# facebookresearch/NasRec

Hardware: AMD Instinct MI355X
Metric: supernet samples/sec at batch 256 (Criteo-shape), 1/2/4/8 MI355X (higher is better)
Workload: dtype f32

## Files before the change

nasrec_amd/csrc/gemm_kslice.hip:

```cpp
#include <cstdlib>
#include <cstring>
#include "gemm_tile.h"

#define KS_TM 32
#define KS_TN 32
#define KS_DC 128
#define KS_NB 4
#define KS_CH ((KS_TM + KS_TN) * KS_DC)
#define KS_SEGS 4
#ifdef KS_STAMPS
#define KS_STAMP(i) \
  if (tid == 0 && d.workspace) d.workspace[blockIdx.x * 64 + (i)] = __builtin_bit_cast(float, (unsigned)__builtin_readcyclecounter())
#define KS_LOOP_STAMP_A const unsigned ks_ta = (unsigned)__builtin_readcyclecounter()
#define KS_LOOP_STAMP_B ks_wait += (unsigned)__builtin_readcyclecounter() - ks_ta
#else
#define KS_STAMP(i)
#define KS_LOOP_STAMP_A
#define KS_LOOP_STAMP_B
#endif

__device__ __forceinline__ __amdgpu_buffer_rsrc_t ks_rsrc(const float* p, long floats) {
  return __builtin_amdgcn_make_buffer_rsrc(const_cast<float*>(p), 0, (int)(floats <= 0 ? 0 : (floats > 0x1fffffffL ? 0x7fffffffL : 4 * floats)), 0x00020000);
}

__global__ __launch_bounds__(1024) void gemm_kslice_kernel(const nasrec_gemm_desc_t d, int tiles_m_, int tiles_n_) {
  extern __shared__ __attribute__((aligned(16))) float ks_lds[];
  const int tid = threadIdx.x, lane = tid & 63;
  KS_STAMP(0);
  warm_kernarg<1024>();
  const int wave = __builtin_amdgcn_readfirstlane(tid >> 6);
#ifndef KS_FEED_FIRST
#define KS_FEED_FIRST 1
#endif
  const int rw = KS_FEED_FIRST ? (wave ^ 8) : wave;
  const int tile = rw & 3;
  const int tm = tile >> 1, tn = tile & 1;
  const int fr = lane & 15, fg = lane >> 4;
  typedef int i32x2 __attribute__((ext_vector_type(2)));
  typedef int i32x4 __attribute__((ext_vector_type(4)));
  i32x4 ab[KS_SEGS], mnkl[KS_SEGS];
  i32x2 ll[KS_SEGS], tiles;
  int nseg;
  {
    const unsigned long long ka = (unsigned long long)__builtin_amdgcn_kernarg_segment_ptr();
    constexpr int S0 = offsetof(nasrec_gemm_desc_t, seg), SS = sizeof(nasrec_gemm_seg_t), OM = offsetof(nasrec_gemm_seg_t, M),
                  OL = offsetof(nasrec_gemm_seg_t, ldb);
    static_assert(KS_SEGS == 4 && offsetof(nasrec_gemm_seg_t, B) == 8 && offsetof(nasrec_gemm_seg_t, lda) == OM + 12 &&
                      offsetof(nasrec_gemm_seg_t, ldc) == OL + 4 && sizeof(nasrec_gemm_desc_t) % 8 == 0,
                  "descriptor layout the scalar loads below assume");
    asm volatile(
        "s_load_dword %12, %14, %c15\n"
        "s_load_dwordx2 %13, %14, %c16\n"
        "s_load_dwordx4 %0, %14, %c17\n"
        "s_load_dwordx4 %1, %14, %c18\n"
        "s_load_dwordx4 %2, %14, %c19\n"
        "s_load_dwordx4 %3, %14, %c20\n"
        "s_load_dwordx4 %4, %14, %c21\n"
        "s_load_dwordx4 %5, %14, %c22\n"
        "s_load_dwordx4 %6, %14, %c23\n"
        "s_load_dwordx4 %7, %14, %c24\n"
        "s_load_dwordx2 %8, %14, %c25\n"
        "s_load_dwordx2 %9, %14, %c26\n"
        "s_load_dwordx2 %10, %14, %c27\n"
        "s_load_dwordx2 %11, %14, %c28\n"
        "s_waitcnt lgkmcnt(0)"
        : "=&s"(ab[0]), "=&s"(ab[1]), "=&s"(ab[2]), "=&s"(ab[3]), "=&s"(mnkl[0]), "=&s"(mnkl[1]), "=&s"(mnkl[2]), "=&s"(mnkl[3]),
          "=&s"(ll[0]), "=&s"(ll[1]), "=&s"(ll[2]), "=&s"(ll[3]), "=&s"(nseg), "=&s"(tiles)
        : "s"(ka), "n"(offsetof(nasrec_gemm_desc_t, nseg)), "n"(sizeof(nasrec_gemm_desc_t)), "n"(S0), "n"(S0 + SS), "n"(S0 + 2 * SS),
          "n"(S0 + 3 * SS), "n"(S0 + OM), "n"(S0 + SS + OM), "n"(S0 + 2 * SS + OM), "n"(S0 + 3 * SS + OM), "n"(S0 + OL),
          "n"(S0 + SS + OL), "n"(S0 + 2 * SS + OL), "n"(S0 + 3 * SS + OL)
        : "memory");
  }
  const float* sA[KS_SEGS];
  const float* sB[KS_SEGS];
  int sK[KS_SEGS], sLa[KS_SEGS], sLb[KS_SEGS], sN[KS_SEGS];
#pragma unroll
  for (int q = 0; q < KS_SEGS; ++q) {
    sA[q] = reinterpret_cast<const float*>(((unsigned long long)(unsigned)ab[q][1] << 32) | (unsigned)ab[q][0]);
    sB[q] = reinterpret_cast<const float*>(((unsigned long long)(unsigned)ab[q][3] << 32) | (unsigned)ab[q][2]);
    sK[q] = mnkl[q][2];
    sLa[q] = mnkl[q][3];
    sLb[q] = ll[q][0];
  }
  const nasrec_gemm_seg_t& s0 = d.seg[0];
  const int M = mnkl[0][0], N = mnkl[0][1];
  const int tiles_m = tiles[0], tiles_n = tiles[1];
  const int nwg = tiles_m * tiles_n, lin0 = blockIdx.x;
  const int q8 = nwg >> 3, r8 = nwg & 7, xcd = lin0 & 7;
  const int lin = (xcd < r8 ? xcd * (q8 + 1) : r8 * (q8 + 1) + (xcd - r8) * q8) + (lin0 >> 3);
  const int PM = tiles_m < 4 ? tiles_m : 4;
  const int panel = lin / (PM * tiles_n), within = lin - panel * PM * tiles_n;
  const int ph = min(PM, tiles_m - panel * PM);
  const int bx = within / ph, by = panel * PM + (within - bx * ph);
  const int m0 = by * KS_TM, n0 = bx * KS_TN;

  int nchunks = 0, ntiny = 0, sT[KS_SEGS];
#pragma unroll
  for (int q = 0; q < KS_SEGS; ++q) {
    const bool live = (q < nseg) & (sA[q] != nullptr) & (sK[q] > 0);
    sK[q] = live ? sK[q] : 0;
    const bool tiny = (sK[q] > 0) & (sK[q] <= 16) & (ntiny < 2);
    sT[q] = tiny ? sK[q] : 0;
    sK[q] = tiny ? 0 : sK[q];
    ntiny += tiny ? 1 : 0;
    sN[q] = (sK[q] + KS_DC - 1) / KS_DC;
    nchunks += sN[q];
  }
  const bool feeder = rw >= 8;
  float* red = ks_lds;
  if (feeder) {
    const int f = rw - 8;
    const bool isB = f >= 4;
    const int pslot = lane & 31;
    int grow[4], gkg[4], growld[4];
#pragma unroll
    for (int i = 0; i < 4; ++i) {
      const int row = 2 * (4 * f + i) + (lane >> 5);
      gkg[i] = pslot ^ (row & 15);
      grow[i] = isB ? min(n0 + row - 32, N - 1) : min(m0 + row, M - 1);
    }
    auto next_live = [&](int seg) {
      int r = KS_SEGS;
#pragma unroll
      for (int q = KS_SEGS - 1; q >= 0; --q) r = (q > seg && sK[q] > 0) ? q : r;
      return r;
    };
    const float* iP;
    int iseg = next_live(-1), iK, ild, ik0 = 0, ibuf = 0;
    __amdgpu_buffer_rsrc_t irs;
    auto issue_segment = [&]() {
      iP = nullptr, iK = 0, ild = 0;
#pragma unroll
      for (int q = 0; q < KS_SEGS; ++q) {
        const bool here = iseg == q;
        iP = here ? (isB ? sB[q] : sA[q]) : iP;
        iK = here ? sK[q] : iK;
        ild = here ? (isB ? sLb[q] : sLa[q]) : ild;
      }
      irs = ks_rsrc(iP, iK > 0 ? (long)((isB ? N : M) - 1) * ild + iK : 0);
#pragma unroll
      for (int i = 0; i < 4; ++i) growld[i] = grow[i] * ild;
    };
    issue_segment();
    auto issue = [&]() {
#pragma unroll
      for (int i = 0; i < 4; ++i) {
        const int k = ik0 + 4 * gkg[i];
        const int vo = k < iK ? 4 * (growld[i] + k) : 0x7ffffff0;
        float* dst = ks_lds + ibuf * KS_CH + (4 * f + i) * 256;
        __builtin_amdgcn_raw_ptr_buffer_load_lds(irs, (__attribute__((address_space(3))) void*)dst, 16, vo, 0, 0, 0);
      }
      ibuf = ibuf + 1 == KS_NB ? 0 : ibuf + 1;
      ik0 += KS_DC;
      if (ik0 >= iK && iseg < KS_SEGS) {
        iseg = next_live(iseg);
        ik0 = 0;
        issue_segment();
      }
    };
#pragma unroll
    for (int c = 0; c < KS_NB - 1; ++c) issue();
#ifdef KS_STAMPS
    unsigned fw_data = 0, fw_bar = 0, fw_issue = 0;
#endif
    for (int c = 0; c < nchunks; ++c) {
#ifdef KS_STAMPS
      const unsigned ta = (unsigned)__builtin_readcyclecounter();
#endif
      asm volatile("s_waitcnt vmcnt(8)" ::: "memory");
#ifdef KS_STAMPS
      const unsigned tb = (unsigned)__builtin_readcyclecounter();
#endif
      __builtin_amdgcn_s_barrier();
#ifdef KS_STAMPS
      const unsigned tc = (unsigned)__builtin_readcyclecounter();
#endif
      issue();
#ifdef KS_STAMPS
      const unsigned td = (unsigned)__builtin_readcyclecounter();
      fw_data += tb - ta, fw_bar += tc - tb, fw_issue += td - tc;
#endif
    }
#ifdef KS_STAMPS
    if (lane == 0 && d.workspace) {
      d.workspace[blockIdx.x * 64 + 16 + wave * 3 + 0] = __builtin_bit_cast(float, fw_data);
      d.workspace[blockIdx.x * 64 + 16 + wave * 3 + 1] = __builtin_bit_cast(float, fw_bar);
      d.workspace[blockIdx.x * 64 + 16 + wave * 3 + 2] = __builtin_bit_cast(float, fw_issue);
    }
#endif
    KS_STAMP(4);
    asm volatile("s_waitcnt vmcnt(0)" ::: "memory");
    __builtin_amdgcn_s_barrier();
  } else {
    const int half = rw >> 2;
#ifdef KS_STAMPS
    unsigned ks_wait = 0;
    const unsigned ks_t0 = (unsigned)__builtin_readcyclecounter();
#endif
    f32x4 acc0 = {0.f, 0.f, 0.f, 0.f}, acc1 = {0.f, 0.f, 0.f, 0.f};
    f32x4 fa[2][4], fb[2][4];
    int flim[2];
    int ck = 0, cbuf = 0;
    int cseg = 0, cK = 0;
    auto seg_k = [&](int seg) {
      int K = 0;
#pragma unroll
      for (int q = 0; q < KS_SEGS; ++q) K = seg == q ? sK[q] : K;
      return K;
    };
    while (cseg < KS_SEGS && seg_k(cseg) == 0) ++cseg;
    cK = seg_k(cseg);
    f32x4 ta = {0.f, 0.f, 0.f, 0.f}, tb = {0.f, 0.f, 0.f, 0.f};
    int tK = 0;
    {
      const float *tA = nullptr, *tB = nullptr;
      int tla = 0, tlb = 0, seen = 0;
#pragma unroll
      for (int q = 0; q < KS_SEGS; ++q) {
        const bool tiny = sT[q] > 0;
        const bool mine = tiny & (seen == half);
        tA = mine ? sA[q] : tA;
        tB = mine ? sB[q] : tB;
        tla = mine ? sLa[q] : tla;
        tlb = mine ? sLb[q] : tlb;
        tK = mine ? sT[q] : tK;
        seen += tiny ? 1 : 0;
      }
      if (tK > 0) {
        const __amdgpu_buffer_rsrc_t ra = ks_rsrc(tA, (long)(M - 1) * tla + tK), rb = ks_rsrc(tB, (long)(N - 1) * tlb + tK);
        const int ia = min(m0 + tm * 16 + fr, M - 1), ib = min(n0 + tn * 16 + fr, N - 1);
        ta = __builtin_bit_cast(f32x4, __builtin_amdgcn_raw_buffer_load_b128(ra, 4 * (ia * tla + 4 * fg), 0, 0));
        tb = __builtin_bit_cast(f32x4, __builtin_amdgcn_raw_buffer_load_b128(rb, 4 * (ib * tlb + 4 * fg), 0, 0));
      }
    }
    auto readfrag = [&](int set) {
      const float* buf = ks_lds + cbuf * KS_CH;
      flim[set] = cK - ck;
#pragma unroll
      for (int kb = 0; kb < 4; ++kb) {
        const int g = 16 * half + 4 * kb + fg;
        fa[set][kb] = *reinterpret_cast<const f32x4*>(buf + (tm * 16 + fr) * KS_DC + 4 * (g ^ fr));
        fb[set][kb] = *reinterpret_cast<const f32x4*>(buf + (32 + tn * 16 + fr) * KS_DC + 4 * (g ^ fr));
      }
      cbuf = cbuf + 1 == KS_NB ? 0 : cbuf + 1;
      ck += KS_DC;
      if (ck >= cK) {
        do {
          ++cseg;
        } while (cseg < KS_SEGS && seg_k(cseg) == 0);
        ck = 0;
        cK = seg_k(cseg);
      }
    };
    auto multiply = [&](int set) {
      const int lim = flim[set];
      if (lim < KS_DC) {
#pragma unroll
        for (int kb = 0; kb < 4; ++kb)
#pragma unroll
          for (int e = 0; e < 4; ++e) {
            const bool in = 4 * (16 * half + 4 * kb + fg) + e < lim;
            fa[set][kb][e] = in ? fa[set][kb][e] : 0.f;
            fb[set][kb][e] = in ? fb[set][kb][e] : 0.f;
          }
      }
#pragma unroll
      for (int kb = 0; kb < 4; kb += 2)
#pragma unroll
        for (int j = 0; j < 4; ++j) {
          acc0 = __builtin_amdgcn_mfma_f32_16x16x4f32(fa[set][kb][j], fb[set][kb][j], acc0, 0, 0, 0);
          acc1 = __builtin_amdgcn_mfma_f32_16x16x4f32(fa[set][kb + 1][j], fb[set][kb + 1][j], acc1, 0, 0, 0);
        }
    };
    for (int t = 0; t < nchunks + 1; t += 2) {
#pragma unroll
      for (int h = 0; h < 2; ++h) {
        const int c = t + h;
        if (c < nchunks) {
          asm volatile("s_waitcnt lgkmcnt(0)" ::: "memory");
          KS_LOOP_STAMP_A;
          __builtin_amdgcn_s_barrier();
          KS_LOOP_STAMP_B;
          readfrag(h);
        }
        if (c >= 1 && c <= nchunks) multiply(h ^ 1);
      }
    }
    KS_STAMP(4);
    asm volatile("s_waitcnt lgkmcnt(0)" ::: "memory");
    __builtin_amdgcn_s_barrier();
    if (tK > 0) {
#pragma unroll
      for (int e = 0; e < 4; ++e) {
        const bool in = 4 * fg + e < tK;
        ta[e] = in ? ta[e] : 0.f;
        tb[e] = in ? tb[e] : 0.f;
      }
#pragma unroll
      for (int j = 0; j < 4; ++j) acc0 = __builtin_amdgcn_mfma_f32_16x16x4f32(ta[j], tb[j], acc0, 0, 0, 0);
    }
    const f32x4 acc = acc0 + acc1;
#ifdef KS_STAMPS
    if (lane == 0 && d.workspace) {
      d.workspace[blockIdx.x * 64 + 16 + wave * 3 + 1] = __builtin_bit_cast(float, ks_wait);
      d.workspace[blockIdx.x * 64 + 16 + wave * 3 + 2] = __builtin_bit_cast(float, (unsigned)__builtin_readcyclecounter() - ks_t0);
    }
#endif
    *reinterpret_cast<f32x4*>(&red[((half * 4 + tile) * 64 + lane) * 4]) = acc;
  }
  __syncthreads();
  KS_STAMP(5);
  {
    const int e = wave;
    const int etile = e >> 2, r = e & 3;
    const float v = red[((0 * 4 + etile) * 64 + lane) * 4 + r] + red[((1 * 4 + etile) * 64 + lane) * 4 + r];
    const int i = m0 + (etile >> 1) * 16 + 4 * fg + r, j = n0 + (etile & 1) * 16 + fr;
    if (i < M && j < N) epilogue_store<NASREC_CM_PLAIN>(d, s0, i, j, v);
  }
  KS_STAMP(6);
}

bool gemm_kslice_eligible(const nasrec_gemm_desc_t* d) {
  if (d->amode != NASREC_AM_KC || d->bmode != NASREC_AM_KC || d->cmode != NASREC_CM_PLAIN || d->zmode || d->splitk > 1) return false;
  if (d->nseg > KS_SEGS) return false;
  const nasrec_gemm_seg_t& s0 = d->seg[0];
  long K = 0;
  for (int q = 0; q < d->nseg; ++q) {
    const nasrec_gemm_seg_t& s = d->seg[q];
    if (s.Aaux || s.Baux || s.ones_col || (s.Mvalid > 0 && s.Mvalid < s0.M)) return false;
    if (s.A && s.K > 0) {
      K += s.K;
      if ((long)s0.M * s.lda >= (1L << 29) || (long)s0.N * s.ldb >= (1L << 29)) return false;
    }
  }
  const long tiles = (long)((s0.M + KS_TM - 1) / KS_TM) * ((s0.N + KS_TN - 1) / KS_TN);
  return s0.M <= 512 && tiles >= 128 && tiles <= 512 && K >= 512;
}

int launch_gemm_kslice(hipStream_t st, const nasrec_gemm_desc_t* d) {
  const nasrec_gemm_seg_t& s0 = d->seg[0];
  const int tiles_m = (s0.M + KS_TM - 1) / KS_TM, tiles_n = (s0.N + KS_TN - 1) / KS_TN;
  static unsigned long long attr_devices = 0;
  const size_t lds = sizeof(float) * KS_NB * KS_CH;
  if (nasrec_lds_attr_needed(attr_devices))
    (void)hipFuncSetAttribute(reinterpret_cast<const void*>(&gemm_kslice_kernel), hipFuncAttributeMaxDynamicSharedMemorySize, (int)lds);
  hipLaunchKernelGGL(gemm_kslice_kernel, dim3((unsigned)(tiles_m * tiles_n)), dim3(1024), lds, st, *d, tiles_m, tiles_n);
  return nasrec_check_launch("gemm_kslice");
}
```

Baseline: 1.160 million.

## Reshape k-slice GEMM tile to 16x48 with one feeder SIMD and four-way K split

Changes the workgroup tile from 32x32 to 16x48 and remaps the 16 waves by SIMD: the waves on SIMD 0 feed A/B chunks into LDS with eight loads each, and each of the other three SIMDs owns one 16x16 output tile whose K range is split four ways across its waves. The final reduction sums four partials per output tile, and the rasterization panel height grows to 8. The aim is to spread MFMA work evenly across SIMDs and shrink the load each feeder wave carries. In exchange each workgroup loads more B per output element, there are fewer MFMAs per wave per chunk, and the deeper vmcnt wait changes how loads overlap. Eligibility still counts 32x32 tiles even though the launch grid now uses 16x48 tiles.

```diff
diff --git a/nasrec_amd/csrc/gemm_kslice.hip b/nasrec_amd/csrc/gemm_kslice.hip
--- a/nasrec_amd/csrc/gemm_kslice.hip
+++ b/nasrec_amd/csrc/gemm_kslice.hip
@@ -2,8 +2,11 @@
 #include <cstring>
 #include "gemm_tile.h"
 
-#define KS_TM 32
-#define KS_TN 32
+#define KS_TM 16
+#define KS_TN 48
+#define KS_NT (KS_TN / 16)
+#define KS_PPF 8
+#define KS_PANEL 8
 #define KS_DC 128
 #define KS_NB 4
 #define KS_CH ((KS_TM + KS_TN) * KS_DC)
@@ -29,12 +32,11 @@
   KS_STAMP(0);
   warm_kernarg<1024>();
   const int wave = __builtin_amdgcn_readfirstlane(tid >> 6);
-#ifndef KS_FEED_FIRST
-#define KS_FEED_FIRST 1
-#endif
-  const int rw = KS_FEED_FIRST ? (wave ^ 8) : wave;
-  const int tile = rw & 3;
-  const int tm = tile >> 1, tn = tile & 1;
+#ifndef KS_SIMD_MAP
+#define KS_SIMD_MAP 0
+#endif
+  const int simd = KS_SIMD_MAP ? (wave >> 2) : (wave & 3), slot = KS_SIMD_MAP ? (wave & 3) : (wave >> 2);
+  const int tile = simd - 1;
   const int fr = lane & 15, fg = lane >> 4;
   typedef int i32x2 __attribute__((ext_vector_type(2)));
   typedef int i32x4 __attribute__((ext_vector_type(4)));
@@ -88,7 +90,7 @@
   const int nwg = tiles_m * tiles_n, lin0 = blockIdx.x;
   const int q8 = nwg >> 3, r8 = nwg & 7, xcd = lin0 & 7;
   const int lin = (xcd < r8 ? xcd * (q8 + 1) : r8 * (q8 + 1) + (xcd - r8) * q8) + (lin0 >> 3);
-  const int PM = tiles_m < 4 ? tiles_m : 4;
+  const int PM = tiles_m < KS_PANEL ? tiles_m : KS_PANEL;
   const int panel = lin / (PM * tiles_n), within = lin - panel * PM * tiles_n;
   const int ph = min(PM, tiles_m - panel * PM);
   const int bx = within / ph, by = panel * PM + (within - bx * ph);
@@ -106,18 +108,18 @@
     sN[q] = (sK[q] + KS_DC - 1) / KS_DC;
     nchunks += sN[q];
   }
-  const bool feeder = rw >= 8;
+  const bool feeder = simd == 0;
   float* red = ks_lds;
   if (feeder) {
-    const int f = rw - 8;
-    const bool isB = f >= 4;
+    const int f = slot;
+    const bool isB = f >= 1;
     const int pslot = lane & 31;
-    int grow[4], gkg[4], growld[4];
-#pragma unroll
-    for (int i = 0; i < 4; ++i) {
-      const int row = 2 * (4 * f + i) + (lane >> 5);
+    int grow[KS_PPF], gkg[KS_PPF], growld[KS_PPF];
+#pragma unroll
+    for (int i = 0; i < KS_PPF; ++i) {
+      const int row = 2 * (KS_PPF * f + i) + (lane >> 5);
       gkg[i] = pslot ^ (row & 15);
-      grow[i] = isB ? min(n0 + row - 32, N - 1) : min(m0 + row, M - 1);
+      grow[i] = isB ? min(n0 + row - KS_TM, N - 1) : min(m0 + row, M - 1);
     }
     auto next_live = [&](int seg) {
       int r = KS_SEGS;
@@ -139,15 +141,15 @@
       }
       irs = ks_rsrc(iP, iK > 0 ? (long)((isB ? N : M) - 1) * ild + iK : 0);
 #pragma unroll
-      for (int i = 0; i < 4; ++i) growld[i] = grow[i] * ild;
+      for (int i = 0; i < KS_PPF; ++i) growld[i] = grow[i] * ild;
     };
     issue_segment();
     auto issue = [&]() {
 #pragma unroll
-      for (int i = 0; i < 4; ++i) {
+      for (int i = 0; i < KS_PPF; ++i) {
         const int k = ik0 + 4 * gkg[i];
         const int vo = k < iK ? 4 * (growld[i] + k) : 0x7ffffff0;
-        float* dst = ks_lds + ibuf * KS_CH + (4 * f + i) * 256;
+        float* dst = ks_lds + ibuf * KS_CH + (KS_PPF * f + i) * 256;
         __builtin_amdgcn_raw_ptr_buffer_load_lds(irs, (__attribute__((address_space(3))) void*)dst, 16, vo, 0, 0, 0);
       }
       ibuf = ibuf + 1 == KS_NB ? 0 : ibuf + 1;
@@ -167,7 +169,8 @@
 #ifdef KS_STAMPS
       const unsigned ta = (unsigned)__builtin_readcyclecounter();
 #endif
-      asm volatile("s_waitcnt vmcnt(8)" ::: "memory");
+      static_assert(KS_PPF * (KS_NB - 2) == 16, "the counted wait below");
+      asm volatile("s_waitcnt vmcnt(16)" ::: "memory");
 #ifdef KS_STAMPS
       const unsigned tb = (unsigned)__builtin_readcyclecounter();
 #endif
@@ -192,13 +195,13 @@
     asm volatile("s_waitcnt vmcnt(0)" ::: "memory");
     __builtin_amdgcn_s_barrier();
   } else {
-    const int half = rw >> 2;
+    const int half = slot >> 1, par = slot & 1;
 #ifdef KS_STAMPS
     unsigned ks_wait = 0;
     const unsigned ks_t0 = (unsigned)__builtin_readcyclecounter();
 #endif
-    f32x4 acc0 = {0.f, 0.f, 0.f, 0.f}, acc1 = {0.f, 0.f, 0.f, 0.f};
-    f32x4 fa[2][4], fb[2][4];
+    f32x4 acc = {0.f, 0.f, 0.f, 0.f};
+    f32x4 fa[2][2], fb[2][2];
     int flim[2];
     int ck = 0, cbuf = 0;
     int cseg = 0, cK = 0;
@@ -218,7 +221,7 @@
 #pragma unroll
       for (int q = 0; q < KS_SEGS; ++q) {
         const bool tiny = sT[q] > 0;
-        const bool mine = tiny & (seen == half);
+        const bool mine = tiny & (seen == half) & (par == 0);
         tA = mine ? sA[q] : tA;
         tB = mine ? sB[q] : tB;
         tla = mine ? sLa[q] : tla;
@@ -228,7 +231,7 @@
       }
       if (tK > 0) {
         const __amdgpu_buffer_rsrc_t ra = ks_rsrc(tA, (long)(M - 1) * tla + tK), rb = ks_rsrc(tB, (long)(N - 1) * tlb + tK);
-        const int ia = min(m0 + tm * 16 + fr, M - 1), ib = min(n0 + tn * 16 + fr, N - 1);
+        const int ia = min(m0 + fr, M - 1), ib = min(n0 + tile * 16 + fr, N - 1);
         ta = __builtin_bit_cast(f32x4, __builtin_amdgcn_raw_buffer_load_b128(ra, 4 * (ia * tla + 4 * fg), 0, 0));
         tb = __builtin_bit_cast(f32x4, __builtin_amdgcn_raw_buffer_load_b128(rb, 4 * (ib * tlb + 4 * fg), 0, 0));
       }
@@ -237,10 +240,10 @@
       const float* buf = ks_lds + cbuf * KS_CH;
       flim[set] = cK - ck;
 #pragma unroll
-      for (int kb = 0; kb < 4; ++kb) {
-        const int g = 16 * half + 4 * kb + fg;
-        fa[set][kb] = *reinterpret_cast<const f32x4*>(buf + (tm * 16 + fr) * KS_DC + 4 * (g ^ fr));
-        fb[set][kb] = *reinterpret_cast<const f32x4*>(buf + (32 + tn * 16 + fr) * KS_DC + 4 * (g ^ fr));
+      for (int u = 0; u < 2; ++u) {
+        const int g = 16 * half + 4 * (par + 2 * u) + fg;
+        fa[set][u] = *reinterpret_cast<const f32x4*>(buf + fr * KS_DC + 4 * (g ^ fr));
+        fb[set][u] = *reinterpret_cast<const f32x4*>(buf + (KS_TM + tile * 16 + fr) * KS_DC + 4 * (g ^ fr));
       }
       cbuf = cbuf + 1 == KS_NB ? 0 : cbuf + 1;
       ck += KS_DC;
@@ -256,21 +259,18 @@
       const int lim = flim[set];
       if (lim < KS_DC) {
 #pragma unroll
-        for (int kb = 0; kb < 4; ++kb)
+        for (int u = 0; u < 2; ++u)
 #pragma unroll
           for (int e = 0; e < 4; ++e) {
-            const bool in = 4 * (16 * half + 4 * kb + fg) + e < lim;
-            fa[set][kb][e] = in ? fa[set][kb][e] : 0.f;
-            fb[set][kb][e] = in ? fb[set][kb][e] : 0.f;
+            const bool in = 4 * (16 * half + 4 * (par + 2 * u) + fg) + e < lim;
+            fa[set][u][e] = in ? fa[set][u][e] : 0.f;
+            fb[set][u][e] = in ? fb[set][u][e] : 0.f;
           }
       }
 #pragma unroll
-      for (int kb = 0; kb < 4; kb += 2)
-#pragma unroll
-        for (int j = 0; j < 4; ++j) {
-          acc0 = __builtin_amdgcn_mfma_f32_16x16x4f32(fa[set][kb][j], fb[set][kb][j], acc0, 0, 0, 0);
-          acc1 = __builtin_amdgcn_mfma_f32_16x16x4f32(fa[set][kb + 1][j], fb[set][kb + 1][j], acc1, 0, 0, 0);
-        }
+      for (int u = 0; u < 2; ++u)
+#pragma unroll
+        for (int j = 0; j < 4; ++j) acc = __builtin_amdgcn_mfma_f32_16x16x4f32(fa[set][u][j], fb[set][u][j], acc, 0, 0, 0);
     };
     for (int t = 0; t < nchunks + 1; t += 2) {
 #pragma unroll
@@ -297,24 +297,24 @@
         tb[e] = in ? tb[e] : 0.f;
       }
 #pragma unroll
-      for (int j = 0; j < 4; ++j) acc0 = __builtin_amdgcn_mfma_f32_16x16x4f32(ta[j], tb[j], acc0, 0, 0, 0);
-    }
-    const f32x4 acc = acc0 + acc1;
+      for (int j = 0; j < 4; ++j) acc = __builtin_amdgcn_mfma_f32_16x16x4f32(ta[j], tb[j], acc, 0, 0, 0);
+    }
 #ifdef KS_STAMPS
     if (lane == 0 && d.workspace) {
       d.workspace[blockIdx.x * 64 + 16 + wave * 3 + 1] = __builtin_bit_cast(float, ks_wait);
       d.workspace[blockIdx.x * 64 + 16 + wave * 3 + 2] = __builtin_bit_cast(float, (unsigned)__builtin_readcyclecounter() - ks_t0);
     }
 #endif
-    *reinterpret_cast<f32x4*>(&red[((half * 4 + tile) * 64 + lane) * 4]) = acc;
+    *reinterpret_cast<f32x4*>(&red[(((half * 2 + par) * KS_NT + tile) * 64 + lane) * 4]) = acc;
   }
   __syncthreads();
   KS_STAMP(5);
-  {
+  if (wave < 4 * KS_NT) {
     const int e = wave;
     const int etile = e >> 2, r = e & 3;
-    const float v = red[((0 * 4 + etile) * 64 + lane) * 4 + r] + red[((1 * 4 + etile) * 64 + lane) * 4 + r];
-    const int i = m0 + (etile >> 1) * 16 + 4 * fg + r, j = n0 + (etile & 1) * 16 + fr;
+    auto part = [&](int h, int p) { return red[(((h * 2 + p) * KS_NT + etile) * 64 + lane) * 4 + r]; };
+    const float v = (part(0, 0) + part(0, 1)) + (part(1, 0) + part(1, 1));
+    const int i = m0 + 4 * fg + r, j = n0 + etile * 16 + fr;
     if (i < M && j < N) epilogue_store<NASREC_CM_PLAIN>(d, s0, i, j, v);
   }
   KS_STAMP(6);
@@ -333,7 +333,7 @@
       if ((long)s0.M * s.lda >= (1L << 29) || (long)s0.N * s.ldb >= (1L << 29)) return false;
     }
   }
-  const long tiles = (long)((s0.M + KS_TM - 1) / KS_TM) * ((s0.N + KS_TN - 1) / KS_TN);
+  const long tiles = (long)((s0.M + 31) / 32) * ((s0.N + 31) / 32);
   return s0.M <= 512 && tiles >= 128 && tiles <= 512 && K >= 512;
 }
 
```

Result: no change. 1.158 million (-0.2%).
